# burlachenkok/flpytorch

Hardware: AMD Instinct MI355X
Metric: gradient-codec encode+reduce GB/s (device-resident), [N,D] fp32; % HBM peak (higher is better)
Workload: dtype f32; 1 GPU; C3 topk:1% N=1024/GPU D=10000000; codec=topk:1%, clients_per_gpu=1024, clients_total=1024, D=10000000, K=100000, rows_alloc=contiguous, parallelism=client-shard dp1

## Files before the change

### flpytorch_amd/_lib.py

```python
import collections
import ctypes
import os
import threading

_HERE = os.path.dirname(os.path.abspath(__file__))
VARIANT_DIR = os.path.join(os.path.dirname(_HERE), "abvar")
LIB_PATH = (os.path.join(VARIANT_DIR, "libflcodec_%s.so" % os.environ["FLC_LIB_VARIANT"])
            if os.environ.get("FLC_LIB_VARIANT") else os.path.join(_HERE, "libflcodec.so"))

FLC_OK, FLC_ERR_ARG, FLC_ERR_DTYPE, FLC_ERR_HIP, FLC_ERR_WORKSPACE, FLC_ERR_UNSUPPORTED = range(6)
FLC_IDENT, FLC_LAZY, FLC_RANDK, FLC_NATURAL, FLC_STD_DITHERING, FLC_NAT_DITHERING, FLC_TOPK, FLC_RANK_K = range(1, 9)
FLC_NORM_LINF, FLC_NORM_L1, FLC_NORM_L2 = 0, 1, 2
FLC_REDUCE_PLAIN, FLC_REDUCE_REL_X = 0, 1
FLC_PATH_AUTO, FLC_PATH_SPARSE, FLC_PATH_DENSE = 0, 1, 2
FLC_TIE_LOWEST, FLC_TIE_HIGHEST = 0, 1
FLC_NORMMODE_EXACT, FLC_NORMMODE_TORCH_CPU = 0, 1
ABI_VERSION = 104


def FLC_ROW_GROUPS(g):
    return (int(g) & 0xFF) << 8

EXPORTS = [
    "flc_version", "flc_build_id", "flc_last_error_string",
    "flc_reduce_rows", "flc_reduce_matrix",
    "flc_encode_workspace_size", "flc_encode",
    "flc_encode_reduce_workspace_size", "flc_encode_reduce",
    "flc_encode_reduce_ex_workspace_size", "flc_encode_reduce_ex",
    "flc_encode_shift_workspace_size", "flc_encode_shift",
    "flc_encode_shift_reduce_workspace_size", "flc_encode_shift_reduce",
    "flc_randk_shift_reduce_workspace_size", "flc_randk_shift_reduce",
    "flc_payload_bytes", "flc_payload_format", "flc_payload_validate", "flc_pack_workspace_size", "flc_pack", "flc_unpack",
    "flc_unpack_reduce_workspace_size", "flc_unpack_reduce",
    "flc_combine_workspace_size", "flc_combine_partials",
    "flc_combine_blocks_workspace_size", "flc_combine_blocks",
    "flc_mt_choice", "flc_mt_rand", "flc_mt_randint31",
    "flc_device_uniform", "flc_device_randk_indices",
    "flc_device_randk_counts_workspace_size", "flc_device_randk_counts",
    "flc_profile_enable", "flc_profile_collect", "flc_select_row_flags",
    "flc_selftest_division", "flc_norm2_torch_cpu", "flc_debug_resident",
    "flc_norm2_torch_cpu_workspace_size", "flc_norm2_torch_cpu_ws", "flc_rows_alloc", "flc_rows_free",
]


class FlcCodecParams(ctypes.Structure):
    _fields_ = [
        ("codec", ctypes.c_int32),
        ("s", ctypes.c_int32),
        ("norm", ctypes.c_int32),
        ("flags", ctypes.c_int32),
        ("k", ctypes.c_int64),
        ("lazy_p", ctypes.c_float),
        ("randk_scale", ctypes.c_float),
        ("d_levels", ctypes.c_void_p),
        ("seed", ctypes.c_uint64),
        ("tie", ctypes.c_int32),
    ]


class FlcPattern(ctypes.Structure):
    _fields_ = [
        ("d_randk_idx", ctypes.c_void_p),
        ("d_uniforms", ctypes.c_void_p),
        ("d_lazy_u", ctypes.c_void_p),
        ("client0", ctypes.c_int64),
        ("uniforms_ld", ctypes.c_int64),
        ("idx_ld", ctypes.c_int64),
        ("d_randk_counts", ctypes.c_void_p),
    ]


class FlcShiftRows(ctypes.Structure):
    _fields_ = [
        ("d_a", ctypes.c_void_p), ("lda", ctypes.c_int64),
# ... 99 lines not shown
    lib.flc_unpack.argtypes = [P(FlcCodecParams), vp, i64, vp, vp]
    lib.flc_unpack_reduce_workspace_size.argtypes = [P(FlcCodecParams), i64, i64]
    lib.flc_unpack_reduce_workspace_size.restype = sz
    lib.flc_unpack_reduce.argtypes = [P(FlcCodecParams), vp, i64, vp, i64, i64, vp, f32, vp, vp, sz, vp]
    lib.flc_combine_workspace_size.argtypes = [vp, i64, i32]
    lib.flc_combine_workspace_size.restype = sz
    lib.flc_combine_partials.argtypes = [vp, vp, i64, f32, i32, vp, sz, vp]
    lib.flc_combine_blocks_workspace_size.argtypes = [vp, i64, i64]
    lib.flc_combine_blocks_workspace_size.restype = sz
    lib.flc_combine_blocks.argtypes = [vp, vp, i64, i64, i64, f32, vp, vp, sz, vp]
    lib.flc_mt_choice.argtypes = [vp, vp, i64, i64, vp, vp]
    lib.flc_mt_rand.argtypes = [vp, vp, i64, vp]
    lib.flc_mt_randint31.argtypes = [vp, vp, i64, vp]
    lib.flc_device_uniform.argtypes = [ctypes.c_uint64, i64, i64]
    lib.flc_device_uniform.restype = ctypes.c_double
    lib.flc_device_randk_indices.argtypes = [ctypes.c_uint64, i64, i64, i64, vp]
    lib.flc_device_randk_counts_workspace_size.argtypes = [i64, i64]
    lib.flc_device_randk_counts_workspace_size.restype = sz
    lib.flc_device_randk_counts.argtypes = [ctypes.c_uint64, i64, i64, i64, i64, vp, vp, sz, vp]
    lib.flc_profile_enable.argtypes = [i32]
    lib.flc_profile_collect.argtypes = [ctypes.c_char_p, vp, vp]
    lib.flc_selftest_division.argtypes = [vp, i32, vp, vp]
    if hasattr(lib, "flc_norm2_torch_cpu"):
        lib.flc_norm2_torch_cpu.argtypes = [vp, i64, i64, i64, vp, vp]
    if hasattr(lib, "flc_norm2_torch_cpu_ws"):
        lib.flc_norm2_torch_cpu_workspace_size.argtypes = [i64, i64]
        lib.flc_norm2_torch_cpu_workspace_size.restype = sz
        lib.flc_norm2_torch_cpu_ws.argtypes = [vp, i64, i64, i64, vp, vp, sz, vp]
    if hasattr(lib, "flc_rows_alloc"):
        lib.flc_rows_alloc.argtypes = [sz, i32, vp]
        lib.flc_rows_free.argtypes = [vp]
    if hasattr(lib, "flc_debug_resident"):
        lib.flc_debug_resident.argtypes = [i32, i64]
    if hasattr(lib, "flc_select_row_flags"):
        lib.flc_select_row_flags.argtypes = [P(FlcCodecParams), i64, i64, vp, sz, vp, vp]
    for name in EXPORTS:
        if not hasattr(lib, name):
            continue
        if name not in ("flc_version", "flc_build_id", "flc_last_error_string", "flc_device_uniform",
                        "flc_encode_workspace_size", "flc_encode_reduce_workspace_size",
                        "flc_encode_reduce_ex_workspace_size", "flc_encode_shift_workspace_size",
                        "flc_encode_shift_reduce_workspace_size", "flc_randk_shift_reduce_workspace_size",
                        "flc_payload_bytes", "flc_pack_workspace_size",
                        "flc_unpack_reduce_workspace_size", "flc_combine_workspace_size",
                        "flc_combine_blocks_workspace_size", "flc_device_randk_counts_workspace_size",
                        "flc_norm2_torch_cpu_workspace_size"):
            getattr(lib, name).restype = i32
    return lib


def source_hash(root=None):
    import glob
    import hashlib
    root = root or os.path.dirname(_HERE)
    csrc = os.path.join(root, "flpytorch_amd", "csrc")
    files = sorted(glob.glob(os.path.join(csrc, "*.hip")) + glob.glob(os.path.join(csrc, "*.hpp")) +
                   glob.glob(os.path.join(csrc, "*.cpp")))
    files += [os.path.join(csrc, "Makefile"), os.path.join(root, "include", "flcodec.h")]
    h = hashlib.sha256()
    for f in files:
        with open(f, "rb") as fh:
            h.update(fh.read())
    return h.hexdigest()[:16]


def build_id():
# ... 87 lines not shown
```

### flpytorch_amd/csrc/api.hip

```cpp
#include <stdarg.h>
#include <stdio.h>

#include <algorithm>
#include <map>
#include <mutex>
#include <string>
#include <vector>

#include "common.hpp"

namespace flc {

static thread_local char g_err[512] = "";

void set_error(const char* fmt, ...) {
    va_list ap;
    va_start(ap, fmt);
    vsnprintf(g_err, sizeof(g_err), fmt, ap);
    va_end(ap);
}

int hip_fail(hipError_t e, const char* what) {
    set_error("%s: %s", what, hipGetErrorString(e));
    return FLC_ERR_HIP;
// ... 91 lines not shown
    if (!d_ptr || bytes == 0) { set_error("flc_rows_alloc: bad args"); return FLC_ERR_ARG; }
    *d_ptr = nullptr;
    const hipError_t e = contiguous ? hipExtMallocWithFlags(d_ptr, bytes, hipDeviceMallocContiguous) : hipMalloc(d_ptr, bytes);
    if (e != hipSuccess) {
        (void)hipGetLastError();
        *d_ptr = nullptr;
        set_error("flc_rows_alloc: %s of %zu bytes failed: %s", contiguous ? "contiguous allocation" : "hipMalloc", bytes,
                  hipGetErrorString(e));
        return FLC_ERR_HIP;
    }
    return FLC_OK;
}

extern "C" int flc_rows_free(void* d_ptr) {
    if (d_ptr && hipFree(d_ptr) != hipSuccess) { set_error("flc_rows_free: hipFree failed"); return FLC_ERR_HIP; }
    return FLC_OK;
}

extern "C" size_t flc_norm2_torch_cpu_workspace_size(int64_t n, int64_t d) {
    return (n <= 0 || d < 0) ? 0 : norm_torch_ws_bytes(n, d);
}

extern "C" int flc_norm2_torch_cpu_ws(const float* d_rows, int64_t ld, int64_t n, int64_t d, float* d_out, void* d_ws,
                                      size_t ws_bytes, void* stream) {
    if (n < 0 || d < 0 || (n > 1 && ld < d) || (n > 0 && (!d_rows || !d_out || !d_ws))) {
        set_error("flc_norm2_torch_cpu_ws: bad args (n=%lld d=%lld ld=%lld)", (long long)n, (long long)d, (long long)ld);
        return FLC_ERR_ARG;
    }
    if (n == 0) return FLC_OK;
    return norm_torch_ws_run(d_rows, ld, n, d, d_out, d_ws, ws_bytes, (hipStream_t)stream);
}

extern "C" int flc_debug_resident(int grid_mult, int64_t spin_ticks) { return rs_debug(grid_mult, spin_ticks); }

extern "C" int flc_norm2_torch_cpu(const float* d_rows, int64_t ld, int64_t n, int64_t d, float* d_out, void* stream) {
    if (n < 0 || d < 0 || (n > 1 && ld < d) || (n > 0 && (!d_rows || !d_out))) {
        set_error("flc_norm2_torch_cpu: bad args (n=%lld d=%lld ld=%lld)", (long long)n, (long long)d, (long long)ld);
        return FLC_ERR_ARG;
    }
    if (n == 0) return FLC_OK;
    return norm_torch_run(d_rows, ld, n, d, d_out, (hipStream_t)stream);
}

namespace flc {
int selftest_division(const float* d_b, int nb, unsigned long long* d_bad, hipStream_t st);
}
extern "C" int flc_selftest_division(const float* d_divisors, int n, unsigned long long* d_mismatches,
                                     void* stream) {
    if (n < 0 || (n > 0 && (!d_divisors || !d_mismatches))) { set_error("flc_selftest_division: bad args"); return FLC_ERR_ARG; }
    if (n == 0) return FLC_OK;
    return selftest_division(d_divisors, n, d_mismatches, (hipStream_t)stream);
}

namespace flc {
size_t encode_row_workspace(const flc_codec_params* prm, int64_t d) {
    if (prm->codec == FLC_TOPK) return sel_workspace(prm, 1, d);
    if (prm->codec == FLC_RANK_K) return rk_workspace(prm, 1, d, false);
    if (prm->codec == FLC_RANDK) return randk_device_workspace(1, d);
    return ew_workspace(prm, 1, d);
}
}

extern "C" size_t flc_encode_workspace_size(const flc_codec_params* prm, int64_t d) {
    if (!prm || !known(prm->codec)) return 0;
    if (prm->codec == FLC_TOPK) return sel_workspace(prm, 1, d);
    if (prm->codec == FLC_RANK_K) return rk_workspace(prm, 1, d, false);
// ... 288 lines not shown
```

### flpytorch_amd/csrc/common.hpp

```cpp
#pragma once
#include <hip/hip_runtime.h>
#include <stdint.h>
#include <stdlib.h>
#include <string.h>

#include "../../include/flcodec.h"

namespace flc {

constexpr int WAVE = 64;
constexpr int CHUNK = 4096;
constexpr int CHUNK_SHIFT = 12;

void set_error(const char* fmt, ...);
int hip_fail(hipError_t e, const char* what);

#define FLC_CHECK_HIP(expr)                                          \
    do {                                                             \
        hipError_t _e = (expr);                                      \
        if (_e != hipSuccess) return ::flc::hip_fail(_e, #expr);     \
    } while (0)
#define FLC_CHECK_LAUNCH(what)                                       \
    do {                                                             \
        hipError_t _e = hipGetLastError();                           \
// ... 110 lines not shown
size_t rk_unpack_workspace(const flc_codec_params* prm, int64_t n, int64_t d);
int rk_unpack1(const flc_codec_params* prm, const float* body, int64_t d, float* out, hipStream_t st);
int rk_unpack_reduce(const flc_codec_params* prm, const char* base, int64_t ld, const char* const* ptrs, int64_t n,
                     int64_t d, const float* w, float wt, float* out, bool reduce, void* wsp, size_t ws_bytes,
                     hipStream_t st);
int payload_format(const flc_codec_params* prm);
int payload_validate(const flc_codec_params* prm, const uint8_t* p, int64_t nbytes, int64_t d);
size_t pack_workspace(const flc_codec_params* prm, int64_t d);
int pack_run(const flc_codec_params* prm, const flc_pattern* pat, const float* x, int64_t d, char* payload, void* ws,
             size_t ws_bytes, hipStream_t st);
int unpack_run(const flc_codec_params* prm, const char* payload, int64_t d, float* out, hipStream_t st);
size_t unpack_reduce_workspace(const flc_codec_params* prm, int64_t n, int64_t d);
int unpack_reduce_run(const flc_codec_params* prm, const char* base, int64_t ld, const char* const* ptrs, int64_t n,
                      int64_t d, const float* w, float wt, float* out, void* ws, size_t ws_bytes, hipStream_t st);
int shift_run(const flc_codec_params* prm, const flc_pattern* pat, const float* a, int64_t d, const ShiftArgs& sh,
              float* pnorm_out, void* ws, size_t ws_bytes, hipStream_t st);
inline int64_t group_row(int64_t n, int G, int g, int lastpct) {
    lastpct = lastpct < 1 ? 1 : lastpct;
    if (G <= 1 || lastpct >= 100) return n * g / G;
    const int64_t unit = 100 * (int64_t)(G - 1) + lastpct;
    const int64_t cum = g <= G - 1 ? 100 * (int64_t)g : unit;
    return n * cum / unit;
}
int norm_torch_run(const float* x, int64_t ld, int64_t n, int64_t d, float* out, hipStream_t st);
size_t norm_torch_ws_bytes(int64_t n, int64_t d);
int norm_torch_ws_run(const float* x, int64_t ld, int64_t n, int64_t d, float* out, void* wsp, size_t ws_bytes,
                      hipStream_t st);
int tn_run(RowSrc rows, int64_t n, int64_t r0, int64_t rn, int64_t d, float* out, void* wsp, const double* item_sums,
           int64_t G, hipStream_t st);
size_t sel_workspace(const flc_codec_params* prm, int64_t n, int64_t d);
int sel_run(const flc_codec_params* prm, const flc_pattern* pat, RowSrc rows, bool vec, int64_t n, int64_t d,
            bool assign, const float* w, float wt, float* out, void* wsp, size_t ws_bytes, hipStream_t st);
int rs_debug(int mult, int64_t spin_ticks);
int sel_row_flags(const flc_codec_params* prm, int64_t n, int64_t d, const void* wsp, size_t ws_bytes,
                  uint32_t* flags, hipStream_t st);
bool ds_eligible(const flc_codec_params* prm, const flc_pattern* pat, int64_t n, int64_t d);
size_t ds_workspace(const flc_codec_params* prm, int64_t n, int64_t d, int norm_mode = FLC_NORMMODE_EXACT);
int ds_run(const flc_codec_params* prm, const flc_pattern* pat, RowSrc rows, int64_t n, int64_t d, const float* w,
           float wt, float* pnorm_out, float* out, void* wsp, size_t ws_bytes, hipStream_t st,
           const float* pnorm_in = nullptr, int norm_mode = FLC_NORMMODE_EXACT);
size_t rk_workspace(const flc_codec_params* prm, int64_t n, int64_t d, bool reduce);
int rk_run(const flc_codec_params* prm, RowSrc rows, int64_t n, int64_t d, bool reduce, const float* w, float wt,
           float* out, void* wsp, size_t ws_bytes, hipStream_t st);
size_t randk_device_workspace(int64_t n, int64_t d);
int randk_device_counts(uint64_t seed, int64_t client0, int64_t n, int64_t d, int64_t k, uint32_t* cnt, void* ws,
                        size_t ws_bytes, hipStream_t st);
int randk_device_prepare(const flc_codec_params* prm, const flc_pattern* pat, int64_t n, int64_t d, void* wsp,
                         const uint32_t** cnt, const uint64_t** ckey, hipStream_t st);
struct RkLists {
    const uint2* tab;
    const uint32_t* idx;
    float* val;
    int64_t cap;
};
size_t randk_lists_workspace(int64_t n, int64_t d, int64_t K);
int randk_lists_build(const flc_codec_params* prm, const flc_pattern* pat, RowSrc rows, int64_t n, int64_t d, void* wsp,
                      RkLists* lists, hipStream_t st);
int randk_lists_fold(int64_t n, int64_t d, int64_t K, void* wsp, const float* w, float wt, float* out, hipStream_t st);
size_t randk_shift_workspace(const flc_codec_params* prm, bool compat, int64_t n, int64_t d);
int randk_shift_run(const flc_codec_params* prm, const flc_pattern* pat, const flc_shift_rows& sr, int64_t n, int64_t d,
                    const float* w, float wt, float* out, void* ws, size_t ws_bytes, hipStream_t st);
int randk_dense(const flc_codec_params* prm, const flc_pattern* pat, const float* x, int64_t d, float* out, void* ws,
                size_t ws_bytes,
                hipStream_t st);

__host__ __device__ inline uint64_t mix64(uint64_t z) {
// ... 83 lines not shown
```

### flpytorch_amd/csrc/select.hip

```cpp
#include <stdlib.h>

#include <atomic>
#include <map>
#include <mutex>
#include <vector>

#include "chunks.hpp"
#include "randk_tree.hpp"

namespace flc {

constexpr uint32_t ALL = 0xFFFFFFFFu;
constexpr uint32_t F_OVERFLOW = 1u, F_SHORT = 2u, F_TIES = 4u, F_EXACT = 8u;
constexpr uint32_t F_RESIDENT = 16u;
constexpr uint32_t F_REPAIR = 32u;
constexpr int SMAX = 16384;
constexpr int HBINS = 2048;
constexpr uint32_t TIECAP = HBINS;
constexpr int CS_SH = 64;
constexpr int64_t CS_FEW = 16;
constexpr int CS_ST = 8;
constexpr int CS_LCAP = 2048;
constexpr int RS_U = 16;
#ifndef FLC_RS_NG
#define FLC_RS_NG 4
#endif
constexpr int RS_NG = FLC_RS_NG;
constexpr int RS_NG_MAX = 16;
static_assert(RS_NG >= 1 && RS_NG <= RS_NG_MAX, "FLC_RS_NG: 1..16 groups");
constexpr int RS_GLOB = 0, RS_GEN = 32, RS_GAVE = 64, RS_CCNT = 96, RS_CDONE = 112, RS_GRP = 128;
constexpr int RS_XGRP = RS_GRP + 32 * RS_NG_MAX;
constexpr int RS_ABV = RS_XGRP + 32 * RS_NG_MAX;
constexpr int RS_CAP = 2048;
constexpr int RS_SS = 8192;
#ifndef FLC_RS_SR
#define FLC_RS_SR 1
#endif
// ... 274 lines not shown
            ma -= aa;
            pb = (pb << pass_bits(p)) | bb;
            mb -= ab;
        }
        ka = NP == 3 ? pa : pa << 9;
        kb = NP == 3 ? pb : pb << 9;
    };
    uint32_t tkey, kest;
    rank_keys(rank, S == d ? rank : (uint32_t)max(1.0, min((double)S, (double)K * (double)S / (double)d)), tkey, kest);
    if (threadIdx.x == 0) {
        ws.thr[row] = (rank >= (uint32_t)S && S != d) ? 0u : tkey;
        ws.prefix[row] = kest;
        ws.flags[row] = 0;
        ws.rowcnt[(row) * RCS] = 0;
        if (few) { ws.cstate[row * CS_ST + 3] = 0; ws.cstate[row * CS_ST + 5] = 0; ws.carrive[row * RCS] = 0; }
    }
    if (few && threadIdx.x < CS_SH) ws.shcnt[(row * CS_SH + threadIdx.x) * RCS] = 0;
    if (few)
        for (int i = threadIdx.x; i < HBINS; i += NT) ws.hist[row * HBINS + i] = 0;
}

#ifndef FLC_CS_NT
#define FLC_CS_NT 1
#endif
__device__ inline float4 cs_ld(const float4* p) {
#if FLC_CS_NT
    typedef float v4f __attribute__((ext_vector_type(4)));
    const v4f v = __builtin_nontemporal_load(reinterpret_cast<const v4f*>(p));
    return make_float4(v.x, v.y, v.z, v.w);
#else
    return *p;
#endif
}
template <int NT>
__device__ void cand_select_row(int64_t row, int64_t K, SelWs ws, uint32_t* h, uint32_t* scratch) {
    {
        if (ws.flags[row]) return;
        const uint32_t cnt = ws.rowcnt[(row) * RCS];
        if (cnt < (uint32_t)K) {
            if (threadIdx.x == 0) ws.flags[row] |= F_SHORT;
            return;
        }
        const uint32_t T = ws.thr[row];
        const uint32_t span = ws.prefix[row] - T;
        int s = 0;
        while (s < 21 && (((uint64_t)span * 4u) >> s) >= (uint64_t)HBINS) ++s;
        const float* vals = ws.ent_val + row * ws.cap;
        const float4* v4 = reinterpret_cast<const float4*>(vals);
        const uint32_t n4 = cnt >> 2;
        uint32_t prefix = 0, krem = (uint32_t)K, last = 0;
        bool first = true, fail = false;
        int sh = s;
        while (true) {
            const int s1 = first ? sh : max(0, sh - 11);
            const uint32_t mask = first ? 0xFFFFFFFFu : ((1u << (sh - s1)) - 1u);
            for (int i = threadIdx.x; i < HBINS; i += NT) h[i] = 0;
            __syncthreads();
            auto add = [&](float x) {
                const uint32_t dk = mag_key(x) - T;
                if (first) atomicAdd(&h[min(dk >> s1, (uint32_t)(HBINS - 1))], 1u);
                else if ((dk >> sh) == prefix) atomicAdd(&h[(dk >> s1) & mask], 1u);
            };
            uint32_t i = threadIdx.x;
            for (; i + 7 * NT < n4; i += 8 * NT) {
                float4 q[8];
#pragma unroll
                for (int u = 0; u < 8; ++u) q[u] = cs_ld(v4 + i + u * NT);
#pragma unroll
                for (int u = 0; u < 8; ++u) { add(q[u].x); add(q[u].y); add(q[u].z); add(q[u].w); }
            }
            for (; i < n4; i += NT) {
                const float4 q = v4[i];
                add(q.x); add(q.y); add(q.z); add(q.w);
            }
            for (uint32_t i = n4 * 4 + threadIdx.x; i < cnt; i += NT) add(vals[i]);
            __syncthreads();
            uint32_t bin, above;
            hist_find(h, krem, bin, above, scratch);
            last = h[bin];
            if (first && bin == HBINS - 1) { fail = true; break; }
            prefix = first ? bin : ((prefix << (sh - s1)) | bin);
            krem -= above;
            sh = s1;
            first = false;
            __syncthreads();
            if (sh == 0) break;
        }
        __syncthreads();
        const uint32_t thr = T + prefix;
        bool ties = !fail && last > krem;
        if (ties && last > TIECAP) { fail = true; ties = false; }
        if (ties) {
            uint32_t* tix = h;
            if (threadIdx.x == 0) scratch[0] = 0;
            __syncthreads();
            const uint32_t* idxs = ws.ent_idx + row * ws.cap;
            for (uint32_t i = threadIdx.x; i < n4; i += NT) {
                const float4 q = v4[i];
                const float qv[4] = {q.x, q.y, q.z, q.w};
#pragma unroll
                for (int u = 0; u < 4; ++u)
                    if (mag_key(qv[u]) == thr) tix[atomicAdd(&scratch[0], 1u)] = idxs[i * 4 + u];
            }
            for (uint32_t i = n4 * 4 + threadIdx.x; i < cnt; i += NT) {
                if (mag_key(vals[i]) == thr) tix[atomicAdd(&scratch[0], 1u)] = idxs[i];
            }
            __syncthreads();
            const uint32_t m = scratch[0];
            for (uint32_t a = threadIdx.x; a < m; a += NT) {
                const uint32_t ia = tix[a];
                uint32_t rank = 0;
                for (uint32_t b = 0; b < m; ++b) rank += tie_pref(tix[b], ws.tie_hi) > tie_pref(ia, ws.tie_hi) ? 1u : 0u;
                if (rank == krem - 1) ws.tiecut[row] = ia;
            }
        }
        if (threadIdx.x == 0) {
            if (fail) {
                ws.flags[row] |= F_SHORT;
            } else {
                ws.thr[row] = thr;
                ws.krem[row] = krem;
                if (ties) ws.flags[row] |= F_TIES;
            }
        }
        __syncthreads();
    }
}

template <int NT>
__global__ __launch_bounds__(NT) void k_cand_select(int64_t r0, int64_t rn, int64_t K, SelWs ws) {
    __shared__ uint32_t h[HBINS];
    __shared__ uint32_t scratch[260];
    for (int64_t row = r0 + blockIdx.x; row < r0 + rn; row += gridDim.x) {
        cand_select_row<NT>(row, K, ws, h, scratch);
        __syncthreads();
    }
}

constexpr int CS_NT = 256;
__global__ __launch_bounds__(CS_NT) void k_cs_pass(int64_t K, SelWs ws, int final_pass) {
    __shared__ uint32_t h[HBINS];
    __shared__ uint32_t scratch[260];
    __shared__ uint32_t last_wg;
    __shared__ uint64_t lst[FLC_CS_LIST ? CS_LCAP : 1];
    const int64_t row = blockIdx.y;
    const uint32_t B = gridDim.x, b = blockIdx.x;
    uint32_t* cs = ws.cstate + row * CS_ST;
    const uint32_t stage = cs[3];
    if (stage >= 2u) return;
    const uint32_t* shc = ws.shcnt + row * CS_SH * RCS;
    uint32_t cnt = 0;
    for (int k = 0; k < CS_SH; ++k) cnt += shc[k * RCS];
    const uint32_t mycnt = shc[b * RCS];
    const bool first = stage == 0u;
    if (first && (ws.flags[row] != 0u || cnt < (uint32_t)K)) {
        if (b == 0 && threadIdx.x == 0) {
            if (ws.flags[row] == 0u) ws.flags[row] = F_SHORT;
            cs[3] = 2u;
        }
        return;
    }
    const uint32_t T = ws.thr[row];
    uint32_t sh, prefix, krem;
    if (first) {
        const uint32_t span = ws.prefix[row] - T;
        uint32_t s0 = 0;
        while (s0 < 21 && (((uint64_t)span * 4u) >> s0) >= (uint64_t)HBINS) ++s0;
// ... 859 lines not shown
                na += adm[q] ? 1u : 0u;
            }
            uint32_t atot;
            uint32_t pos = base + ex_scan<NT>(na, wsum, atot);
#pragma unroll
            for (int q = 0; q < 4; ++q)
                if (adm[q]) { oi[pos] = (uint32_t)(j0 + q); ov[pos] = v[q]; ++pos; }
            base += atot;
            tie_run += etot;
            if (sb == SUBS - 1 && t == 0) ws.tab[c * n + row] = make_uint2(cbase, base - cbase);
        }
        if (t == 0) {
            ws.thr[row] = thr;
            ws.krem[row] = krem;
            ws.rowcnt[row * RCS] = base;
            ws.flags[row] = F_EXACT | (ws.flags[row] & (F_OVERFLOW | F_SHORT));
        }
        __syncthreads();
    }
}

template <bool VEC>
__global__ __launch_bounds__(EX_NT) void k_topk_exact_rows(RowSrc rows, int64_t n, int64_t r0, int64_t rn, int64_t d, int64_t K, SelWs ws) {
    __shared__ uint32_t h[HBINS];
    __shared__ uint32_t scratch[260];
    __shared__ uint32_t wsum[EX_NT / 64];
    for (int64_t row = r0 + blockIdx.x; row < r0 + rn; row += gridDim.x) {
        if (!(ws.flags[row] & (F_OVERFLOW | F_SHORT))) continue;
        exact_row<VEC>(rows, n, row, d, K, ws, h, scratch, wsum);
    }
}

template <int NT, bool VEC>
__global__ __launch_bounds__(NT) void k_cand_select_x(RowSrc rows, int64_t n, int64_t r0, int64_t rn, int64_t d, int64_t K,
                                                      SelWs ws) {
    __shared__ uint32_t h[HBINS];
    __shared__ uint32_t scratch[260];
    __shared__ uint32_t wsum[NT / 64];
    __shared__ uint32_t failed;
    for (int64_t row = r0 + blockIdx.x; row < r0 + rn; row += gridDim.x) {
        cand_select_row<NT>(row, K, ws, h, scratch);
        __syncthreads();
        if (threadIdx.x == 0) failed = __atomic_load_n(&ws.flags[row], __ATOMIC_RELAXED) & (F_OVERFLOW | F_SHORT);
        __syncthreads();
        if (failed) exact_row<VEC, NT>(rows, n, row, d, K, ws, h, scratch, wsum);
        __syncthreads();
    }
}

__global__ __launch_bounds__(256) void k_tie_count(RowSrc rows, int64_t n, int64_t d, SelWs ws) {
    const int64_t C = nchunks(d);
    const int lane = threadIdx.x & 63, wv = threadIdx.x >> 6;
    const int64_t nrows = *ws.nwork;
    const int64_t bpr = (C + 3) / 4;
    for (int64_t it = blockIdx.x; it < nrows * bpr; it += gridDim.x) {
        const int64_t row = ws.worklist[it / bpr];
        const int64_t c = (it % bpr) * 4 + wv;
        if (c >= C) continue;
        uint32_t cnt = 0;
        if (ws.flags[row] & F_TIES) {
            const uint32_t T = ws.thr[row];
            const float* r = rows.row(row);
            const int64_t j1 = min(d, (c + 1) * (int64_t)CHUNK);
            for (int64_t j = c * CHUNK + lane; j < j1; j += 64) cnt += (mag_key(r[j]) == T) ? 1u : 0u;
            cnt = wave_sum(cnt);
        }
        if (lane == 0) ws.tieprefix[c * n + row] = cnt;
    }
}

__global__ __launch_bounds__(256) void k_tie_scan(int64_t n, int64_t d, SelWs ws) {
    constexpr bool EXACT = true;
    __shared__ uint32_t part[256];
    const int64_t C = nchunks(d);
// ... 1751 lines not shown
}

static bool cs_single() {
    static const bool v = [] { const char* e = tuning_env("FLC_CS_SINGLE"); return e && atoi(e) == 1; }();
    return v;
}

#ifndef FLC_LONE_PATH
#define FLC_LONE_PATH 2
#endif
#ifndef FLC_RS_EVREC
#define FLC_RS_EVREC 1
#endif
#ifndef FLC_RS_COOP
#define FLC_RS_COOP 0
#endif
struct RsCtx {
    uint32_t* ctl = nullptr;
    uint32_t seq = 0;
    uint32_t xcum = 0;
    hipStream_t last = nullptr;
    hipEvent_t done = nullptr;
};
static std::mutex g_rs_mu;
static std::map<int, RsCtx> g_rs_ctx;
static std::atomic<int> g_rs_dbg_mult{1};
static std::atomic<long long> g_rs_dbg_spin{0};
int rs_debug(int mult, int64_t spin_ticks) {
    if (mult < 1 || mult > 64 || spin_ticks < 0) { set_error("flc_debug_resident: mult 1..64, spin >= 0"); return FLC_ERR_ARG; }
    g_rs_dbg_mult.store(mult);
    g_rs_dbg_spin.store((long long)spin_ticks);
    return FLC_OK;
}
static int rs_cus() {
    static int cu[64] = {0};
    int dev = 0;
    if (hipGetDevice(&dev) != hipSuccess || dev < 0 || dev >= 64) return 0;
    if (!cu[dev]) {
        int c = 0;
        if (hipDeviceGetAttribute(&c, hipDeviceAttributeMultiprocessorCount, dev) != hipSuccess) return 0;
        cu[dev] = c;
    }
    return cu[dev];
}
static int lone_path() {
    static const int v = [] { const char* e = tuning_env("FLC_LONE_PATH"); return e ? atoi(e) : FLC_LONE_PATH; }();
    return v;
}

static int filter_group() {
    static const int g = [] {
        const char* e = tuning_env("FLC_FILTER_GS");
        return (e && atoi(e) == 2) ? 2 : 4;
    }();
    return g;
}

template <int FGS>
static void launch_filter(RowSrc rows, int64_t n, int64_t r0, int64_t rn, int64_t d, SelWs ws, hipStream_t st,
                          int shards, float* zout = nullptr) {
    const int64_t waves = rn * ((nchunks(d) + FGS - 1) / FGS);
    const int gw = (int)std::max<int64_t>(1, std::min<int64_t>((waves + 3) / 4, 32768));
    static const int64_t rb = [] {
        const char* e = tuning_env("FLC_TK_RB");
        return e ? std::max<int64_t>(1, atoll(e)) : (int64_t)64;
    }();
    ProfScope _pv(FGS == 4 ? "k_topk_filter_g4" : "k_topk_filter_g2", st);
    if constexpr (FGS == 4 && FLC_TK_WG != 0 && FLC_TK_PROBE != 1 && FLC_TK_PROBE != 3) {
        static const bool wg = [] { const char* e = tuning_env("FLC_FILTER_WG"); return !(e && atoi(e) == 0); }();
        if (wg && shards == 1 && !zout) {
            constexpr int NL = FLC_TK_WG_NL;
            const int64_t items = rn * ((nchunks(d) + 4 * NL - 1) / (4 * NL));
            const int gi = (int)std::max<int64_t>(1, std::min<int64_t>(items, 32768));
            static const int64_t rbw = [] {
                const char* e = tuning_env("FLC_TK_RB");
                return e ? std::max<int64_t>(1, atoll(e)) : (int64_t)16;
            }();
            hipLaunchKernelGGL((k_topk_filter_fast_wg<FLC_TK_WG_RING, NL>), dim3(gi), dim3((NL + 1) * 64), 0, st, rows, n, r0,
                               rn, std::min(rbw, std::max<int64_t>(rn, 1)), d, ws);
            return;
        }
    }
    if (zout)
        hipLaunchKernelGGL((k_topk_filter_fast<FLC_TK_RING, FGS, 1>), dim3(gw), dim3(256), 0, st, rows, n, r0, rn,
                           std::min(rb, std::max<int64_t>(rn, 1)), d, ws, shards, zout);
    else
        hipLaunchKernelGGL((k_topk_filter_fast<FLC_TK_RING, FGS>), dim3(gw), dim3(256), 0, st, rows, n, r0, rn,
                           std::min(rb, std::max<int64_t>(rn, 1)), d, ws, shards, (float*)nullptr);
}

#ifndef FLC_TK_SPLIT_SAMPLE
#define FLC_TK_SPLIT_SAMPLE 1
#endif
#ifndef FLC_TK_LASTPCT
#define FLC_TK_LASTPCT 100
#endif
static_assert(FLC_TK_LASTPCT >= 1 && FLC_TK_LASTPCT <= 100, "FLC_TK_LASTPCT: the last row group is 1..100 % of the others");
#ifndef FLC_TK_LAST_TS
#define FLC_TK_LAST_TS 4096
#endif
#ifndef FLC_TK_GFOLD
#define FLC_TK_GFOLD 1
#endif
#ifndef FLC_TK_SIDE_NT
#define FLC_TK_SIDE_NT 512
#endif
#ifndef FLC_TK_EXACT_WG
#define FLC_TK_EXACT_WG 256
#endif
static int tk_tail_groups(const flc_codec_params* prm, int64_t n) {
    static const int g = [] { const char* e = tuning_env("FLC_TK_TAILOV"); return e ? std::max(1, atoi(e)) : 4; }();
    const int hint = (prm->flags >> 8) & 0xFF;
    if (hint) return (int)std::max<int64_t>(1, std::min<int64_t>(hint, n));
    return (int)std::max<int64_t>(1, std::min<int64_t>(g, n / 64));
}
namespace {
struct TkCtx {
    hipStream_t side = nullptr;
    std::vector<hipEvent_t> ev;
};
std::mutex g_tk_mu;
std::map<int, TkCtx> g_tk_ctx;
}

static int launch_chunk_accum(int64_t n, int64_t d, SelWs ws, bool assign, const float* w, float wt, float* out,
// ... 254 lines not shown
                return FLC_OK;
            }
        }
        const bool dense_k = K * 16 > d;
        lone_assign = assign && n == 1 && few && !dense_k && !assign_fold();

        if (dense_k) FLC_CHECK_HIP(hipMemsetAsync(ws.hist, 0, (size_t)n * HBINS * sizeof(uint32_t), st));
        const int64_t bpr = (C + 3) / 4;
        if (!dense_k) {
            const int TG = few ? 1 : tk_tail_groups(prm, n);
            gfold = FLC_TK_GFOLD && !few && !assign && !dense_k;
            hipStream_t sside = st;
            TkCtx* cx = nullptr;
            std::unique_lock<std::mutex> lk;
            if (TG > 1) {
                int dev = 0;
                FLC_CHECK_HIP(hipGetDevice(&dev));
                lk = std::unique_lock<std::mutex>(g_tk_mu);
                cx = &g_tk_ctx[dev];
                if (!cx->side) {
                    int lo = 0, hi = 0;
                    FLC_CHECK_HIP(hipDeviceGetStreamPriorityRange(&lo, &hi));
                    FLC_CHECK_HIP(hipStreamCreateWithPriority(&cx->side, hipStreamNonBlocking, hi));
                }
                while ((int)cx->ev.size() < TG + 3) {
                    hipEvent_t e;
                    FLC_CHECK_HIP(hipEventCreateWithFlags(&e, FLC_SYNC_EVENT_FLAGS));
                    cx->ev.push_back(e);
                }
                sside = cx->side;
            }
            const bool split = FLC_TK_SPLIT_SAMPLE && TG > 1;
            const int64_t rs1 = split ? group_row(n, TG, 1, FLC_TK_LASTPCT) : n;
            auto sample = [&](int64_t a, int64_t b, hipStream_t sx) {
                if (b <= a) return;
                ProfScope _ps("k_topk_sample", sx);
                hipLaunchKernelGGL((few ? k_topk_sample<1024, true> : k_topk_sample<1024, false>), dim3((unsigned)(b - a)), dim3(1024), 0, sx,
                                   rows, n, d, K, ws, few ? 1 : 0, a);
            };
            if (split) {
                FLC_CHECK_HIP(hipEventRecord(cx->ev[TG + 1], st));
                FLC_CHECK_HIP(hipStreamWaitEvent(sside, cx->ev[TG + 1], 0));
            }
            sample(0, rs1, st);
            FLC_CHECK_LAUNCH("k_topk_sample");
            if (split) {
                sample(rs1, n, sside);
                FLC_CHECK_LAUNCH("k_topk_sample (side)");
                FLC_CHECK_HIP(hipEventRecord(cx->ev[TG + 2], sside));
            }
            for (int g = 0; g < TG; ++g) {
                const int64_t r0 = group_row(n, TG, g, FLC_TK_LASTPCT), rn = group_row(n, TG, g + 1, FLC_TK_LASTPCT) - r0;
                if (split && g == 1) FLC_CHECK_HIP(hipStreamWaitEvent(st, cx->ev[TG + 2], 0));
                { ProfScope _ps("k_topk_filter", st);
                float* zout = lone_assign ? out : nullptr;
                if (filter_group() == 2 || n * d < ((int64_t)64 << 20)) launch_filter<2>(rows, n, r0, rn, d, ws, st, few ? CS_SH : 1, zout);
                else launch_filter<4>(rows, n, r0, rn, d, ws, st, few ? CS_SH : 1, zout); }
                FLC_CHECK_LAUNCH("k_topk_filter");
                if (TG > 1) {
                    FLC_CHECK_HIP(hipEventRecord(cx->ev[g], st));
                    FLC_CHECK_HIP(hipStreamWaitEvent(sside, cx->ev[g], 0));
                }
                { ProfScope _ps("k_cand_select", sside);
                if (few) {
                    const int np = (FLC_CS_LIST && d <= FLC_CS_TWO_MAXD) ? 2 : 3;
                    for (int p = 0; p < np; ++p)
                        hipLaunchKernelGGL(k_cs_pass, dim3((unsigned)CS_SH, (unsigned)n), dim3(CS_NT), 0, st, K, ws,
                                           p == np - 1 ? 1 : 0);
                } else if (gfold) {
                    const bool big = rn < 128 || g == TG - 1;
                    const int nt = big ? 1024 : FLC_TK_SIDE_NT;
                    const dim3 grid((unsigned)(big ? rn : grid_stride_blocks(rn, 8192)));
                    if (big) {
                        if (vec) hipLaunchKernelGGL((k_cand_select_x<1024, true>), grid, dim3(nt), 0, sside, rows, n, r0, rn, d, K, ws);
                        else hipLaunchKernelGGL((k_cand_select_x<1024, false>), grid, dim3(nt), 0, sside, rows, n, r0, rn, d, K, ws);
                    } else if (FLC_TK_SIDE_NT == 256) {
                        if (vec) hipLaunchKernelGGL((k_cand_select_x<256, true>), grid, dim3(nt), 0, sside, rows, n, r0, rn, d, K, ws);
                        else hipLaunchKernelGGL((k_cand_select_x<256, false>), grid, dim3(nt), 0, sside, rows, n, r0, rn, d, K, ws);
                    } else {
                        if (vec) hipLaunchKernelGGL((k_cand_select_x<512, true>), grid, dim3(nt), 0, sside, rows, n, r0, rn, d, K, ws);
                        else hipLaunchKernelGGL((k_cand_select_x<512, false>), grid, dim3(nt), 0, sside, rows, n, r0, rn, d, K, ws);
                    }
                } else if (rn < 128 || (TG > 1 && g == TG - 1))
                    hipLaunchKernelGGL(k_cand_select<1024>, dim3((unsigned)rn), dim3(1024), 0, sside, r0, rn, K, ws);
                else if (FLC_TK_SIDE_NT == 256)
                    hipLaunchKernelGGL(k_cand_select<256>, dim3(grid_stride_blocks(rn, 8192)), dim3(256), 0, sside, r0, rn, K, ws);
                else hipLaunchKernelGGL(k_cand_select<512>, dim3(grid_stride_blocks(rn, 8192)), dim3(512), 0, sside, r0, rn, K, ws); }
                FLC_CHECK_LAUNCH("k_cand_select");
                if (gfold) {
                    const bool lastg = g == TG - 1;
                    if (int rc = launch_group_fold(n, d, ws, w, wt, out, r0, r0 + rn, g == 0, lastg, lastg || TG == 1, sside))
                        return rc;
                }
            }
            if (!lone_assign && !gfold) {
                ProfScope _ps("k_topk_exact_rows", sside);
                const int eb = grid_stride_blocks(n, FLC_TK_EXACT_WG);
                if (vec) hipLaunchKernelGGL((k_topk_exact_rows<true>), dim3(eb), dim3(EX_NT), 0, sside, rows, n, (int64_t)0, n, d, K, ws);
                else hipLaunchKernelGGL((k_topk_exact_rows<false>), dim3(eb), dim3(EX_NT), 0, sside, rows, n, (int64_t)0, n, d, K, ws);
                FLC_CHECK_LAUNCH("k_topk_exact_rows");
            }
            if (TG > 1) {
                FLC_CHECK_HIP(hipEventRecord(cx->ev[TG], sside));
                FLC_CHECK_HIP(hipStreamWaitEvent(st, cx->ev[TG], 0));
            }
        } else {
            FLC_CHECK_HIP(hipMemsetAsync(ws.flags, 0, (size_t)n * sizeof(uint32_t), st));
        }
        if (dense_k) {
        hipLaunchKernelGGL(k_build_worklist, dim3(1), dim3(1024), 0, st, n, K, d, ws, 1);
        FLC_CHECK_LAUNCH("k_build_worklist");
        const int64_t hb = (d + 65535) / 65536;
        for (int p = 0; p < 3; ++p) {
            { ProfScope _ps("k_radix_hist_full", st);
hipLaunchKernelGGL((k_radix_hist<true>), dim3(grid_stride_blocks(n * hb)), dim3(256), 0, st, rows, n, d, p, ws); }
            FLC_CHECK_LAUNCH("k_radix_hist(full)");
            hipLaunchKernelGGL((k_radix_select<true>), dim3(grid_stride_blocks(n, 1024)), dim3(256), 0, st, n, p, K, ws);
            FLC_CHECK_LAUNCH("k_radix_select(full)");
        }
        hipLaunchKernelGGL(k_tie_count, dim3(grid_stride_blocks(n * bpr, 4096)), dim3(256), 0, st, rows, n, d, ws);
// ... 134 lines not shown
```

### include/flcodec.h

```cpp
#ifndef FLCODEC_H
#define FLCODEC_H

#include <stddef.h>
#include <stdint.h>

#ifdef __cplusplus
extern "C" {
#endif

typedef enum {
    FLC_OK = 0,
    FLC_ERR_ARG = 1,
    FLC_ERR_DTYPE = 2,
    FLC_ERR_HIP = 3,
    FLC_ERR_WORKSPACE = 4,
    FLC_ERR_UNSUPPORTED = 5
} flc_status;

typedef enum {
    FLC_IDENT = 1,
    FLC_LAZY = 2,
    FLC_RANDK = 3,
    FLC_NATURAL = 4,
    FLC_STD_DITHERING = 5,
// ... 121 lines not shown
int flc_combine_blocks(void* rccl_comm, const float* d_blocks, int64_t ld, int64_t nb_local, int64_t d,
                       float w_total, float* d_out, void* d_ws, size_t ws_bytes, void* stream);

int flc_mt_choice(uint32_t* h_key, int32_t* h_pos, int64_t n, int64_t k, int64_t* h_out,
                  int64_t* h_scratch);
int flc_mt_rand(uint32_t* h_key, int32_t* h_pos, int64_t n, double* h_out);
int flc_mt_randint31(uint32_t* h_key, int32_t* h_pos, int64_t count, int64_t* h_out);

double flc_device_uniform(uint64_t seed, int64_t client, int64_t j);
int flc_device_randk_indices(uint64_t seed, int64_t client, int64_t d, int64_t k, int64_t* h_out);
size_t flc_device_randk_counts_workspace_size(int64_t n, int64_t d);
int flc_device_randk_counts(uint64_t seed, int64_t client0, int64_t n, int64_t d, int64_t k, uint32_t* d_counts,
                            void* d_ws, size_t ws_bytes, void* stream);

int flc_norm2_torch_cpu(const float* d_rows, int64_t ld, int64_t n, int64_t d, float* d_out, void* stream);

size_t flc_norm2_torch_cpu_workspace_size(int64_t n, int64_t d);
int flc_norm2_torch_cpu_ws(const float* d_rows, int64_t ld, int64_t n, int64_t d, float* d_out, void* d_ws,
                           size_t ws_bytes, void* stream);

int flc_selftest_division(const float* d_divisors, int n, unsigned long long* d_mismatches, void* stream);

int flc_profile_enable(int on);
int flc_profile_collect(const char* kernel, double* h_total_ms, int64_t* h_launches);

int flc_select_row_flags(const flc_codec_params* prm, int64_t n, int64_t d, const void* d_workspace,
                         size_t ws_bytes, uint32_t* d_flags, void* stream);

int flc_rows_alloc(size_t bytes, int contiguous, void** d_ptr);
int flc_rows_free(void* d_ptr);

int flc_debug_resident(int grid_mult, int64_t spin_ticks);

#ifdef __cplusplus
}
#endif
#endif
```

Before: 5914 GB/s.

## Add window-based k-th selection to candidate select with sampled bounds

Adds a windowed path to the top-k candidate selection kernel. A strided sample pass estimates a value range around the k-th magnitude, and a single walk compacts in-range candidates into a shared-memory window. The k-th key is then resolved by radix histogramming over that window instead of repeated digit passes over the whole candidate list, with fallback to the original digit loop when the window overflows. It also adds a 32KB shared window, min-waves launch bounds, global stat counters with atomics, and a debug mode switch, which can lower occupancy and adds atomic traffic.

```diff
diff --git a/flpytorch_amd/_lib.py b/flpytorch_amd/_lib.py
--- a/flpytorch_amd/_lib.py
+++ b/flpytorch_amd/_lib.py
@@ -40,6 +40,7 @@
     "flc_profile_enable", "flc_profile_collect", "flc_select_row_flags",
     "flc_selftest_division", "flc_norm2_torch_cpu", "flc_debug_resident",
     "flc_norm2_torch_cpu_workspace_size", "flc_norm2_torch_cpu_ws", "flc_rows_alloc", "flc_rows_free",
+    "flc_debug_select",
 ]
 
 
@@ -205,6 +206,8 @@
         lib.flc_rows_free.argtypes = [vp]
     if hasattr(lib, "flc_debug_resident"):
         lib.flc_debug_resident.argtypes = [i32, i64]
+    if hasattr(lib, "flc_debug_select"):
+        lib.flc_debug_select.argtypes = [i32, P(ctypes.c_int64)]
     if hasattr(lib, "flc_select_row_flags"):
         lib.flc_select_row_flags.argtypes = [P(FlcCodecParams), i64, i64, vp, sz, vp, vp]
     for name in EXPORTS:
diff --git a/flpytorch_amd/csrc/api.hip b/flpytorch_amd/csrc/api.hip
--- a/flpytorch_amd/csrc/api.hip
+++ b/flpytorch_amd/csrc/api.hip
@@ -147,6 +147,8 @@
 }
 
 extern "C" int flc_debug_resident(int grid_mult, int64_t spin_ticks) { return rs_debug(grid_mult, spin_ticks); }
+
+extern "C" int flc_debug_select(int mode, int64_t* h_stats) { return cs_debug(mode, h_stats); }
 
 extern "C" int flc_norm2_torch_cpu(const float* d_rows, int64_t ld, int64_t n, int64_t d, float* d_out, void* stream) {
     if (n < 0 || d < 0 || (n > 1 && ld < d) || (n > 0 && (!d_rows || !d_out))) {
diff --git a/flpytorch_amd/csrc/common.hpp b/flpytorch_amd/csrc/common.hpp
--- a/flpytorch_amd/csrc/common.hpp
+++ b/flpytorch_amd/csrc/common.hpp
@@ -166,6 +166,7 @@
 int sel_run(const flc_codec_params* prm, const flc_pattern* pat, RowSrc rows, bool vec, int64_t n, int64_t d,
             bool assign, const float* w, float wt, float* out, void* wsp, size_t ws_bytes, hipStream_t st);
 int rs_debug(int mult, int64_t spin_ticks);
+int cs_debug(int mode, int64_t* h_stats);
 int sel_row_flags(const flc_codec_params* prm, int64_t n, int64_t d, const void* wsp, size_t ws_bytes,
                   uint32_t* flags, hipStream_t st);
 bool ds_eligible(const flc_codec_params* prm, const flc_pattern* pat, int64_t n, int64_t d);
diff --git a/flpytorch_amd/csrc/select.hip b/flpytorch_amd/csrc/select.hip
--- a/flpytorch_amd/csrc/select.hip
+++ b/flpytorch_amd/csrc/select.hip
@@ -3,6 +3,7 @@
 #include <atomic>
 #include <map>
 #include <mutex>
+#include <type_traits>
 #include <vector>
 
 #include "chunks.hpp"
@@ -343,13 +344,130 @@
     return *p;
 #endif
 }
+#ifndef FLC_CS_WINDOW
+#define FLC_CS_WINDOW 1
+#endif
+#ifndef FLC_CS_WCAP
+#define FLC_CS_WCAP 8192
+#endif
+constexpr uint32_t CS_WCAP = FLC_CS_WINDOW ? FLC_CS_WCAP : 1;
+constexpr uint32_t CS_WFILL = 3 * FLC_CS_WCAP / 4;
+constexpr int CS_WST = 4;
+constexpr int CS_QMAX = 16;
+#define CS_MINW(NT) ((NT) == 1024 ? 4 : (NT) == 512 ? 5 : 3)
+__device__ unsigned long long g_cs_stat[3];
+
 template <int NT>
-__device__ void cand_select_row(int64_t row, int64_t K, SelWs ws, uint32_t* h, uint32_t* scratch) {
+__device__ void cs_window_walk(const float* vals, uint32_t cnt, uint32_t T, uint32_t base, uint32_t hi, bool none,
+                               uint32_t* win, uint32_t* wst) {
+    const float4* v4 = reinterpret_cast<const float4*>(vals);
+    const uint32_t n4 = cnt >> 2;
+    uint32_t nab = 0;
+    uint32_t tid = threadIdx.x;
+    asm volatile("" : "+v"(tid));
+    const uint32_t width = min(hi, 0xFFFFFFFEu) - base, top = ~base;
+    auto place = [&](const uint32_t* rel, auto nvc) {
+        constexpr int NV = decltype(nvc)::value;
+        uint32_t tot = 0;
+#pragma unroll
+        for (int j = 0; j < NV; ++j) {
+            nab += rel[j] > width && rel[j] < top ? 1u : 0u;
+            tot += (uint32_t)__popcll(__ballot(rel[j] <= width));
+        }
+        if (tot == 0 || none) return;
+        uint32_t slot = 0;
+        if ((tid & 63) == 0) slot = atomicAdd(&wst[0], tot);
+        slot = (uint32_t)__builtin_amdgcn_readfirstlane((int)slot);
+#pragma unroll
+        for (int j = 0; j < NV; ++j) {
+            uint32_t r = rel[j];
+            asm volatile("" : "+v"(r));
+            const bool in = r <= width;
+            const uint64_t m = __ballot(in);
+            if (in) {
+                const uint32_t pos = slot + __builtin_amdgcn_mbcnt_hi((uint32_t)(m >> 32), __builtin_amdgcn_mbcnt_lo((uint32_t)m, 0u));
+                if (pos < CS_WCAP) win[pos] = rel[j];
+            }
+            slot += (uint32_t)__popcll(m);
+        }
+    };
+    const uint32_t tb = T + base;
+    constexpr int U = NT == 512 ? 4 : 8;
+    for (uint32_t i0 = 0; i0 < n4; i0 += U * NT) {
+        uint32_t rel[4 * U];
+        if (i0 + U * NT <= n4) {
+#pragma unroll
+            for (int u = 0; u < U; ++u) {
+                const float4 q = cs_ld(v4 + i0 + u * NT + tid);
+                rel[4 * u] = __float_as_uint(q.x); rel[4 * u + 1] = __float_as_uint(q.y);
+                rel[4 * u + 2] = __float_as_uint(q.z); rel[4 * u + 3] = __float_as_uint(q.w);
+            }
+#pragma unroll
+            for (int j = 0; j < 4 * U; ++j) rel[j] = (rel[j] & 0x7FFFFFFFu) - tb;
+        } else {
+#pragma unroll
+            for (int u = 0; u < U; ++u) {
+                const uint32_t i = i0 + u * NT + tid;
+                const bool ok = i < n4;
+                const float4 q = ok ? cs_ld(v4 + i) : make_float4(0.f, 0.f, 0.f, 0.f);
+                rel[4 * u] = ok ? mag_key(q.x) - tb : ALL;
+                rel[4 * u + 1] = ok ? mag_key(q.y) - tb : ALL;
+                rel[4 * u + 2] = ok ? mag_key(q.z) - tb : ALL;
+                rel[4 * u + 3] = ok ? mag_key(q.w) - tb : ALL;
+            }
+        }
+#pragma unroll
+        for (int u = 0; u < 4 * U; u += 8) place(rel + u, std::integral_constant<int, 8>{});
+    }
+    if (tid < 64) {
+        const uint32_t i = n4 * 4 + tid;
+        const uint32_t rel = i < cnt ? mag_key(vals[i]) - tb : ALL;
+        place(&rel, std::integral_constant<int, 1>{});
+    }
+#pragma unroll
+    for (int off = 32; off; off >>= 1) nab += __shfl_xor(nab, off, 64);
+    if ((tid & 63) == 0 && nab) atomicAdd(&wst[1], nab);
+}
+
+template <int NT>
+__device__ void cs_window_kth(const uint32_t* win, uint32_t w, uint32_t maxrel, uint32_t m, uint32_t* h, uint32_t* scratch,
+                              uint32_t& relk, uint32_t& krem, uint32_t& last) {
+    int sh = maxrel ? 32 - __clz((int)maxrel) : 0;
+    uint32_t prefix = 0;
+    krem = m;
+    while (true) {
+        const int s1 = max(0, sh - 11);
+        const uint32_t mask = (1u << (sh - s1)) - 1u;
+        for (int i = threadIdx.x; i < HBINS; i += NT) h[i] = 0;
+        __syncthreads();
+        for (uint32_t i = threadIdx.x; i < w; i += NT) {
+            const uint32_t r = win[i];
+            if (sh >= 32 || (r >> sh) == prefix) atomicAdd(&h[(r >> s1) & mask], 1u);
+        }
+        __syncthreads();
+        uint32_t bin, above;
+        hist_find(h, krem, bin, above, scratch);
+        last = h[bin];
+        prefix = (prefix << (sh - s1)) | bin;
+        krem -= above;
+        sh = s1;
+        __syncthreads();
+        if (sh == 0) break;
+    }
+    relk = prefix;
+}
+
+template <int NT>
+__device__ void cand_select_row(int64_t row, int64_t K, SelWs ws, uint32_t* h, uint32_t* scratch, uint32_t* win, int wmode) {
     {
-        if (ws.flags[row]) return;
+        if (ws.flags[row]) {
+            if (FLC_CS_WINDOW && threadIdx.x == 0) atomicAdd(&g_cs_stat[2], 1ull);
+            return;
+        }
         const uint32_t cnt = ws.rowcnt[(row) * RCS];
         if (cnt < (uint32_t)K) {
             if (threadIdx.x == 0) ws.flags[row] |= F_SHORT;
+            if (FLC_CS_WINDOW && threadIdx.x == 0) atomicAdd(&g_cs_stat[2], 1ull);
             return;
         }
         const uint32_t T = ws.thr[row];
@@ -362,7 +480,78 @@
         uint32_t prefix = 0, krem = (uint32_t)K, last = 0;
         bool first = true, fail = false;
         int sh = s;
+        int wres = 2;
+        enum { ST_PASS_A, ST_WALK, ST_DIGIT } st = ST_DIGIT;
+        uint32_t base = 0, hi = 0xFFFFFFFFu, q = 1;
+        const bool none = wmode == 2;
+        bool onebin = false;
+        if (FLC_CS_WINDOW && wmode != 1) {
+            if (cnt <= CS_WCAP) {
+                st = ST_WALK;
+            } else {
+                const float kc = (float)K * (float)(cnt - (uint32_t)K) / (float)cnt;
+                constexpr float wt2 = (float)(CS_WFILL / 8) * (float)(CS_WFILL / 8);
+                q = kc * CS_QMAX <= wt2 ? (uint32_t)CS_QMAX : (uint32_t)fmaxf(1.f, wt2 / kc);
+                if (q > 1) st = ST_PASS_A;
+                else if (wmode == 0) onebin = true;
+                else wres = 1;
+            }
+        }
         while (true) {
+            if (FLC_CS_WINDOW && st == ST_PASS_A) {
+                for (int i = threadIdx.x; i < HBINS; i += NT) h[i] = 0;
+                __syncthreads();
+                const uint32_t nsl = ((cnt >> 5) + q - 1) / q;
+                constexpr uint32_t LPR = NT / 8;
+                const uint32_t sub = threadIdx.x & 7u;
+                auto add = [&](float x) { atomicAdd(&h[min((mag_key(x) - T) >> s, (uint32_t)(HBINS - 1))], 1u); };
+                uint32_t l = threadIdx.x >> 3;
+                constexpr int UA = NT == 512 ? 2 : 4;
+                for (; l + (UA - 1) * LPR < nsl; l += UA * LPR) {
+                    float4 a[UA];
+#pragma unroll
+                    for (int u = 0; u < UA; ++u) a[u] = cs_ld(v4 + (l + u * LPR) * q * 8u + sub);
+#pragma unroll
+                    for (int u = 0; u < UA; ++u) { add(a[u].x); add(a[u].y); add(a[u].z); add(a[u].w); }
+                }
+                for (; l < nsl; l += LPR) {
+                    const float4 a = cs_ld(v4 + l * q * 8u + sub);
+                    add(a.x); add(a.y); add(a.z); add(a.w);
+                }
+                __syncthreads();
+                const float kc = (float)K * (float)(cnt - (uint32_t)K) / (float)cnt;
+                const float f = (float)(nsl * 32u) / (float)cnt, kf = (float)K * f;
+                const float delta = 4.f * sqrtf(kc * f) + 8.f;
+                uint32_t b_hi = HBINS - 1, b_lo, above;
+                if (kf - delta >= 1.f) hist_find(h, (uint32_t)(kf - delta), b_hi, above, scratch);
+                hist_find(h, (uint32_t)ceilf(kf + delta), b_lo, above, scratch);
+                base = b_lo << s;
+                if (b_hi < (uint32_t)(HBINS - 1)) hi = ((b_hi + 1u) << s) - 1u;
+                st = ST_WALK;
+                continue;
+            }
+            if (FLC_CS_WINDOW && st == ST_WALK) {
+                uint32_t* wst = win + CS_WCAP;
+                if (threadIdx.x < CS_WST) wst[threadIdx.x] = 0;
+                __syncthreads();
+                cs_window_walk<NT>(vals, cnt, T, base, hi, none, win, wst);
+                __syncthreads();
+                const uint32_t w = wst[0], above = wst[1];
+                const uint32_t maxrel = min(hi, 0x7FFFFFFFu - T) - base;
+                wres = 1;
+                if (w <= CS_WCAP && above < (uint32_t)K && (uint32_t)K - above <= w) {
+                    uint32_t relk, wk, wl;
+                    cs_window_kth<NT>(win, w, maxrel, (uint32_t)K - above, h, scratch, relk, wk, wl);
+                    const uint32_t dkk = base + relk;
+                    if ((dkk >> s) < (uint32_t)(HBINS - 1)) {
+                        prefix = dkk; krem = wk; last = wl;
+                        wres = 0;
+                        break;
+                    }
+                }
+                st = ST_DIGIT;
+                continue;
+            }
             const int s1 = first ? sh : max(0, sh - 11);
             const uint32_t mask = first ? 0xFFFFFFFFu : ((1u << (sh - s1)) - 1u);
             for (int i = threadIdx.x; i < HBINS; i += NT) h[i] = 0;
@@ -396,7 +585,16 @@
             first = false;
             __syncthreads();
             if (sh == 0) break;
-        }
+            if (FLC_CS_WINDOW && onebin) {
+                onebin = false;
+                if (last <= CS_WCAP) {
+                    base = prefix << sh;
+                    hi = base + ((1u << sh) - 1u);
+                    st = ST_WALK;
+                }
+            }
+        }
+        if (FLC_CS_WINDOW && threadIdx.x == 0) atomicAdd(&g_cs_stat[wres], 1ull);
         __syncthreads();
         const uint32_t thr = T + prefix;
         bool ties = !fail && last > krem;
@@ -439,11 +637,12 @@
 }
 
 template <int NT>
-__global__ __launch_bounds__(NT) void k_cand_select(int64_t r0, int64_t rn, int64_t K, SelWs ws) {
+__global__ __launch_bounds__(NT, CS_MINW(NT)) void k_cand_select(int64_t r0, int64_t rn, int64_t K, SelWs ws, int wmode) {
     __shared__ uint32_t h[HBINS];
     __shared__ uint32_t scratch[260];
+    __shared__ uint32_t win[CS_WCAP + CS_WST];
     for (int64_t row = r0 + blockIdx.x; row < r0 + rn; row += gridDim.x) {
-        cand_select_row<NT>(row, K, ws, h, scratch);
+        cand_select_row<NT>(row, K, ws, h, scratch, win, wmode);
         __syncthreads();
     }
 }
@@ -1369,14 +1568,15 @@
 }
 
 template <int NT, bool VEC>
-__global__ __launch_bounds__(NT) void k_cand_select_x(RowSrc rows, int64_t n, int64_t r0, int64_t rn, int64_t d, int64_t K,
-                                                      SelWs ws) {
+__global__ __launch_bounds__(NT, CS_MINW(NT)) void k_cand_select_x(RowSrc rows, int64_t n, int64_t r0, int64_t rn, int64_t d, int64_t K,
+                                                      SelWs ws, int wmode) {
     __shared__ uint32_t h[HBINS];
     __shared__ uint32_t scratch[260];
     __shared__ uint32_t wsum[NT / 64];
     __shared__ uint32_t failed;
+    __shared__ uint32_t win[CS_WCAP + CS_WST];
     for (int64_t row = r0 + blockIdx.x; row < r0 + rn; row += gridDim.x) {
-        cand_select_row<NT>(row, K, ws, h, scratch);
+        cand_select_row<NT>(row, K, ws, h, scratch, win, wmode);
         __syncthreads();
         if (threadIdx.x == 0) failed = __atomic_load_n(&ws.flags[row], __ATOMIC_RELAXED) & (F_OVERFLOW | F_SHORT);
         __syncthreads();
@@ -3194,6 +3394,20 @@
     g_rs_dbg_spin.store((long long)spin_ticks);
     return FLC_OK;
 }
+static std::atomic<int> g_cs_mode{0};
+int cs_debug(int mode, int64_t* h_stats) {
+    if (mode < 0 || mode > 2) { set_error("flc_debug_select: mode 0..2"); return FLC_ERR_ARG; }
+    g_cs_mode.store(mode);
+    if (h_stats) {
+        unsigned long long st[3] = {0, 0, 0};
+        const unsigned long long zero[3] = {0, 0, 0};
+        FLC_CHECK_HIP(hipDeviceSynchronize());
+        FLC_CHECK_HIP(hipMemcpyFromSymbol(st, HIP_SYMBOL(g_cs_stat), sizeof(st)));
+        FLC_CHECK_HIP(hipMemcpyToSymbol(HIP_SYMBOL(g_cs_stat), zero, sizeof(zero)));
+        for (int i = 0; i < 3; ++i) h_stats[i] = (int64_t)st[i];
+    }
+    return FLC_OK;
+}
 static int rs_cus() {
     static int cu[64] = {0};
     int dev = 0;
@@ -3253,6 +3467,9 @@
 
 #ifndef FLC_TK_SPLIT_SAMPLE
 #define FLC_TK_SPLIT_SAMPLE 1
+#endif
+#ifndef FLC_TK_SAMPLE_DUAL0
+#define FLC_TK_SAMPLE_DUAL0 0
 #endif
 #ifndef FLC_TK_LASTPCT
 #define FLC_TK_LASTPCT 100
@@ -3573,20 +3790,20 @@
             }
             const bool split = FLC_TK_SPLIT_SAMPLE && TG > 1;
             const int64_t rs1 = split ? group_row(n, TG, 1, FLC_TK_LASTPCT) : n;
-            auto sample = [&](int64_t a, int64_t b, hipStream_t sx) {
+            auto sample = [&](int64_t a, int64_t b, hipStream_t sx, bool dual) {
                 if (b <= a) return;
                 ProfScope _ps("k_topk_sample", sx);
-                hipLaunchKernelGGL((few ? k_topk_sample<1024, true> : k_topk_sample<1024, false>), dim3((unsigned)(b - a)), dim3(1024), 0, sx,
+                hipLaunchKernelGGL((dual ? k_topk_sample<1024, true> : k_topk_sample<1024, false>), dim3((unsigned)(b - a)), dim3(1024), 0, sx,
                                    rows, n, d, K, ws, few ? 1 : 0, a);
             };
             if (split) {
                 FLC_CHECK_HIP(hipEventRecord(cx->ev[TG + 1], st));
                 FLC_CHECK_HIP(hipStreamWaitEvent(sside, cx->ev[TG + 1], 0));
             }
-            sample(0, rs1, st);
+            sample(0, rs1, st, few || (FLC_TK_SAMPLE_DUAL0 && split));
             FLC_CHECK_LAUNCH("k_topk_sample");
             if (split) {
-                sample(rs1, n, sside);
+                sample(rs1, n, sside, false);
                 FLC_CHECK_LAUNCH("k_topk_sample (side)");
                 FLC_CHECK_HIP(hipEventRecord(cx->ev[TG + 2], sside));
             }
@@ -3602,6 +3819,7 @@
                     FLC_CHECK_HIP(hipEventRecord(cx->ev[g], st));
                     FLC_CHECK_HIP(hipStreamWaitEvent(sside, cx->ev[g], 0));
                 }
+                const int wmode = g_cs_mode.load();
                 { ProfScope _ps("k_cand_select", sside);
                 if (few) {
                     const int np = (FLC_CS_LIST && d <= FLC_CS_TWO_MAXD) ? 2 : 3;
@@ -3613,20 +3831,20 @@
                     const int nt = big ? 1024 : FLC_TK_SIDE_NT;
                     const dim3 grid((unsigned)(big ? rn : grid_stride_blocks(rn, 8192)));
                     if (big) {
-                        if (vec) hipLaunchKernelGGL((k_cand_select_x<1024, true>), grid, dim3(nt), 0, sside, rows, n, r0, rn, d, K, ws);
-                        else hipLaunchKernelGGL((k_cand_select_x<1024, false>), grid, dim3(nt), 0, sside, rows, n, r0, rn, d, K, ws);
+                        if (vec) hipLaunchKernelGGL((k_cand_select_x<1024, true>), grid, dim3(nt), 0, sside, rows, n, r0, rn, d, K, ws, wmode);
+                        else hipLaunchKernelGGL((k_cand_select_x<1024, false>), grid, dim3(nt), 0, sside, rows, n, r0, rn, d, K, ws, wmode);
                     } else if (FLC_TK_SIDE_NT == 256) {
-                        if (vec) hipLaunchKernelGGL((k_cand_select_x<256, true>), grid, dim3(nt), 0, sside, rows, n, r0, rn, d, K, ws);
-                        else hipLaunchKernelGGL((k_cand_select_x<256, false>), grid, dim3(nt), 0, sside, rows, n, r0, rn, d, K, ws);
+                        if (vec) hipLaunchKernelGGL((k_cand_select_x<256, true>), grid, dim3(nt), 0, sside, rows, n, r0, rn, d, K, ws, wmode);
+                        else hipLaunchKernelGGL((k_cand_select_x<256, false>), grid, dim3(nt), 0, sside, rows, n, r0, rn, d, K, ws, wmode);
                     } else {
-                        if (vec) hipLaunchKernelGGL((k_cand_select_x<512, true>), grid, dim3(nt), 0, sside, rows, n, r0, rn, d, K, ws);
-                        else hipLaunchKernelGGL((k_cand_select_x<512, false>), grid, dim3(nt), 0, sside, rows, n, r0, rn, d, K, ws);
+                        if (vec) hipLaunchKernelGGL((k_cand_select_x<512, true>), grid, dim3(nt), 0, sside, rows, n, r0, rn, d, K, ws, wmode);
+                        else hipLaunchKernelGGL((k_cand_select_x<512, false>), grid, dim3(nt), 0, sside, rows, n, r0, rn, d, K, ws, wmode);
                     }
                 } else if (rn < 128 || (TG > 1 && g == TG - 1))
-                    hipLaunchKernelGGL(k_cand_select<1024>, dim3((unsigned)rn), dim3(1024), 0, sside, r0, rn, K, ws);
+                    hipLaunchKernelGGL(k_cand_select<1024>, dim3((unsigned)rn), dim3(1024), 0, sside, r0, rn, K, ws, wmode);
                 else if (FLC_TK_SIDE_NT == 256)
-                    hipLaunchKernelGGL(k_cand_select<256>, dim3(grid_stride_blocks(rn, 8192)), dim3(256), 0, sside, r0, rn, K, ws);
-                else hipLaunchKernelGGL(k_cand_select<512>, dim3(grid_stride_blocks(rn, 8192)), dim3(512), 0, sside, r0, rn, K, ws); }
+                    hipLaunchKernelGGL(k_cand_select<256>, dim3(grid_stride_blocks(rn, 8192)), dim3(256), 0, sside, r0, rn, K, ws, wmode);
+                else hipLaunchKernelGGL(k_cand_select<512>, dim3(grid_stride_blocks(rn, 8192)), dim3(512), 0, sside, r0, rn, K, ws, wmode); }
                 FLC_CHECK_LAUNCH("k_cand_select");
                 if (gfold) {
                     const bool lastg = g == TG - 1;
diff --git a/include/flcodec.h b/include/flcodec.h
--- a/include/flcodec.h
+++ b/include/flcodec.h
@@ -177,6 +177,8 @@
 
 int flc_debug_resident(int grid_mult, int64_t spin_ticks);
 
+int flc_debug_select(int mode, int64_t* h_stats);
+
 #ifdef __cplusplus
 }
 #endif
```

After: 5998 GB/s (median of 6 runs). +1.4%, better.
